# adobe/3D-FM-GAN

Measured on AMD Instinct MI355X. Metric: (photo,render) pairs/sec, higher is better.
Workload: dtype f32; 1 GPU; pairs1024: cfg4 shard: E_Tsr+E_W+E_W_Plus(18 styles) on 256^2 -> co-mod -> Generator(1024) forward, fp32, B=8/GPU; pairs_per_gpu=8, global_pairs=8, image_size=1024, parallelism=replicas x1 (batch-sharded, no collective), launch=eager, ranks=1, full=False

## Files before the change

3d-fm-gan_amd/csrc/live_weights.hip:

```cpp
#include "common.h"

namespace {

constexpr int LW_TO = 64, LW_TI = 16, LW_MAXT = 9;
constexpr int LW_ELEMS0 = 2048;

__global__ __launch_bounds__(256) void live_weights_f32(const fmgan_refresh_entry* __restrict__ table, int n_entries) {
  __shared__ float tile[LW_TO][LW_TI * LW_MAXT + 1];
  int lo = 0, hi = n_entries - 1;
  while (lo < hi) {
    const int mid = (lo + hi + 1) >> 1;
    if (table[mid].block_begin <= blockIdx.x) lo = mid; else hi = mid - 1;
  }
  const fmgan_refresh_entry e = table[lo];
  const unsigned lb = blockIdx.x - e.block_begin;
  const float* __restrict__ src = (const float*)e.src;
  float* __restrict__ dst = (float*)e.dst;
  if (e.kind == 0) {
    const long long base = (long long)lb * LW_ELEMS0;
#pragma unroll
    for (int k = 0; k < LW_ELEMS0 / 256; ++k) {
      const long long idx = base + threadIdx.x + 256 * k;
      if (idx < e.n) dst[idx] = src[idx] * e.scale;
    }
    return;
  }
  const int kt = e.ktaps, run = LW_TI * kt;
  const int i_tiles = (e.cin + LW_TI - 1) / LW_TI;
  const int o0 = (lb / i_tiles) * LW_TO, i0 = (lb % i_tiles) * LW_TI;
  const int i_n = min(LW_TI, e.cin - i0);
  for (int idx = threadIdx.x; idx < LW_TO * run; idx += 256) {
    const int o = idx / run, j = idx - o * run;
    float v = 0.f;
    if (o0 + o < e.cout && j < i_n * kt) v = src[((long long)(o0 + o) * e.cin + i0) * kt + j];
    tile[o][j] = v;
  }
  __syncthreads();
  for (int idx = threadIdx.x; idx < LW_TO * run; idx += 256) {
    const int j = idx / LW_TO, o = idx - j * LW_TO;
    if (o0 + o < e.cout && j < i_n * kt) dst[((long long)i0 * kt + j) * e.cout + o0 + o] = e.scale * tile[o][j];
  }
  float* __restrict__ wsq = (float*)e.dst2;
  if (wsq) {
    for (int idx = threadIdx.x; idx < LW_TO * LW_TI; idx += 256) {
      const int o = idx / LW_TI, i = idx % LW_TI;
      if (o0 + o < e.cout && i < i_n) {
        float q = 0.f;
        for (int t = 0; t < kt; ++t) { const float w = tile[o][i * kt + t]; q = fmaf(w, w, q); }
        wsq[(long long)(o0 + o) * e.cin + i0 + i] = q;
      }
    }
  }
}

}

extern "C" long long fmgan_weight_refresh_blocks(int kind, int cout, int cin, int ktaps, long long n) {
  if (kind == 0) return n > 0 ? (n + LW_ELEMS0 - 1) / LW_ELEMS0 : -1;
  if (kind == 1) {
    if (cout <= 0 || cin <= 0 || ktaps <= 0 || ktaps > LW_MAXT) return -1;
    return (long long)((cout + LW_TO - 1) / LW_TO) * ((cin + LW_TI - 1) / LW_TI);
  }
  return -1;
}

extern "C" int fmgan_weight_refresh_f32(const fmgan_refresh_entry* table_dev, int n_entries, long long total_blocks,
                                        void* stream) {
  if (n_entries < 0 || total_blocks < 0) return FMGAN_EINVAL;
  if (n_entries == 0 || total_blocks == 0) return FMGAN_OK;
  if (!table_dev) return FMGAN_EINVAL;
  if (total_blocks > 0x7fffffffLL) return FMGAN_EOVERFLOW;
  hipLaunchKernelGGL(live_weights_f32, dim3((unsigned)total_blocks), dim3(256), 0, (hipStream_t)stream, table_dev,
                     n_entries);
  return fmgan_check_launch();
}
```

3d-fm-gan_amd/csrc/winograd.hip:

```cpp
#include "common.h"

namespace {

__global__ __launch_bounds__(256) void wino_weight_f32(const float* __restrict__ wt, float* __restrict__ u, int cin, int cout) {
  const long long total = (long long)cin * cout;
  for (long long idx = (long long)blockIdx.x * blockDim.x + threadIdx.x; idx < total; idx += (long long)gridDim.x * blockDim.x) {
    const int i = (int)(idx % cin), o = (int)(idx / cin);
    float g[3][3];
#pragma unroll
    for (int t = 0; t < 9; ++t) g[t / 3][t % 3] = wt[((long long)i * 9 + t) * cout + o];
    float tmp[4][3];
#pragma unroll
    for (int k = 0; k < 3; ++k) {
      tmp[0][k] = g[0][k];
      tmp[1][k] = 0.5f * (g[0][k] + g[1][k] + g[2][k]);
      tmp[2][k] = 0.5f * (g[0][k] - g[1][k] + g[2][k]);
      tmp[3][k] = g[2][k];
    }
#pragma unroll
    for (int a = 0; a < 4; ++a) {
      const float uu[4] = {tmp[a][0], 0.5f * (tmp[a][0] + tmp[a][1] + tmp[a][2]), 0.5f * (tmp[a][0] - tmp[a][1] + tmp[a][2]),
                           tmp[a][2]};
#pragma unroll
      for (int bx = 0; bx < 4; ++bx) u[((long long)(a * 4 + bx) * cout + o) * cin + i] = uu[bx];
    }
  }
}

__global__ __launch_bounds__(256) void wino_input_f32(const float* __restrict__ x, const float* __restrict__ style,
                                                      float* __restrict__ v, int batch, int c, int h, int w) {
  const int tw = w >> 1, th = h >> 1, T = tw * th;
  const long long n_cols = (long long)batch * T, total = n_cols * c;
  for (long long idx = (long long)blockIdx.x * blockDim.x + threadIdx.x; idx < total; idx += (long long)gridDim.x * blockDim.x) {
    const int t = (int)(idx % T);
    const int ch = (int)((idx / T) % c);
    const int b = (int)(idx / ((long long)T * c));
    const int ty = t / tw, tx = t - ty * tw;
    const float* xp = x + ((long long)b * c + ch) * h * w;
    const float s = style[(long long)b * c + ch];
    float d[4][4];
#pragma unroll
    for (int r = 0; r < 4; ++r) {
      const int y = 2 * ty - 1 + r;
#pragma unroll
      for (int q = 0; q < 4; ++q) {
        const int xx = 2 * tx - 1 + q;
        d[r][q] = (y >= 0 && y < h && xx >= 0 && xx < w) ? xp[(long long)y * w + xx] * s : 0.f;
      }
    }
    float e[4][4];
#pragma unroll
    for (int r = 0; r < 4; ++r) {
      e[r][0] = d[r][0] - d[r][2]; e[r][1] = d[r][1] + d[r][2]; e[r][2] = d[r][2] - d[r][1]; e[r][3] = d[r][1] - d[r][3];
    }
    const long long col = (long long)b * T + t;
#pragma unroll
    for (int q = 0; q < 4; ++q) {
      const float v0 = e[0][q] - e[2][q], v1 = e[1][q] + e[2][q], v2 = e[2][q] - e[1][q], v3 = e[1][q] - e[3][q];
// ... 20 lines not shown
    const int ty = t / tw, tx = t - ty * tw;
    const long long col = (long long)b * T + t;
    float mm[4][4];
#pragma unroll
    for (int a = 0; a < 4; ++a)
#pragma unroll
      for (int q = 0; q < 4; ++q) mm[a][q] = m[((long long)(a * 4 + q) * cout + o) * n_cols + col];
    float z[2][4];
#pragma unroll
    for (int q = 0; q < 4; ++q) {
      z[0][q] = mm[0][q] + mm[1][q] + mm[2][q];
      z[1][q] = mm[1][q] - mm[2][q] - mm[3][q];
    }
    const float dm = demod ? demod[(long long)b * cout + o] : 1.f;
    const float bv = (fuse_act && bias) ? bias[o] : 0.f;
    float* op = out + (((long long)b * cout + o) * h + 2 * ty) * w + 2 * tx;
    const float* np = (fuse_act && noise) ? noise + ((long long)(noise_batch == 1 ? 0 : b) * h + 2 * ty) * w + 2 * tx : nullptr;
#pragma unroll
    for (int jy = 0; jy < 2; ++jy) {
      float y0 = (z[jy][0] + z[jy][1] + z[jy][2]) * dm, y1 = (z[jy][1] - z[jy][2] - z[jy][3]) * dm;
      if (fuse_act) {
        const float n0 = np ? __fmul_rn(nw, np[jy * w]) : 0.f, n1 = np ? __fmul_rn(nw, np[jy * w + 1]) : 0.f;
        y0 = __fadd_rn(__fadd_rn(y0, n0), bv);
        y1 = __fadd_rn(__fadd_rn(y1, n1), bv);
        y0 = (y0 > 0.f ? y0 : y0 * alpha) * act_scale;
        y1 = (y1 > 0.f ? y1 : y1 * alpha) * act_scale;
      }
      f32x2_u st; st.x = y0; st.y = y1;
      *reinterpret_cast<f32x2_u*>(op + (long long)jy * w) = st;
    }
  }
}

inline unsigned wino_grid(long long total) {
  long long blocks = (total + 255) / 256;
  const long long cap = (long long)FMGAN_NUM_CU * 32;
  if (blocks > cap) blocks = cap;
  return (unsigned)(blocks < 1 ? 1 : blocks);
}

}

extern "C" int fmgan_wino_weight_f32(const float* wt, float* u, int cin, int cout, void* stream) {
  if (cin <= 0 || cout <= 0) return FMGAN_EINVAL;
  if (!wt || !u) return FMGAN_EINVAL;
  hipLaunchKernelGGL(wino_weight_f32, dim3(wino_grid((long long)cin * cout)), dim3(256), 0, (hipStream_t)stream, wt, u, cin, cout);
  return fmgan_check_launch();
}

extern "C" int fmgan_wino_input_f32(const float* x, const float* style, float* v, int batch, int c, int h, int w, void* stream) {
  if (batch < 0 || c <= 0 || h <= 0 || w <= 0 || (h & 1) || (w & 1)) return FMGAN_EINVAL;
  if (batch == 0) return FMGAN_OK;
  if (!x || !style || !v) return FMGAN_EINVAL;
  hipLaunchKernelGGL(wino_input_f32, dim3(wino_grid((long long)batch * c * (h / 2) * (w / 2))), dim3(256), 0, (hipStream_t)stream,
                     x, style, v, batch, c, h, w);
  return fmgan_check_launch();
}

extern "C" int fmgan_wino_output_f32(const float* m, const float* demod, const float* noise, const float* noise_weight,
                                     const float* bias, float* out, int batch, int cout, int h, int w, int noise_batch,
                                     int fuse_act, float alpha, float act_scale, void* stream) {
  if (batch < 0 || cout <= 0 || h <= 0 || w <= 0 || (h & 1) || (w & 1)) return FMGAN_EINVAL;
  if (batch == 0) return FMGAN_OK;
  if (!m || !out) return FMGAN_EINVAL;
  if (fuse_act && noise && noise_batch != 1 && noise_batch != batch) return FMGAN_EINVAL;
  hipLaunchKernelGGL(wino_output_f32, dim3(wino_grid((long long)batch * cout * (h / 2) * (w / 2))), dim3(256), 0,
                     (hipStream_t)stream, m, demod, noise, noise_weight, bias, out, batch, cout, h, w, noise_batch, fuse_act, alpha,
                     act_scale);
  return fmgan_check_launch();
}
```

3d-fm-gan_amd/op/_native/__init__.py:

```python
from .core import (
    LIB_PATH, F32, F64, F16, BF16, FMGAN_OK, FMGAN_EINVAL, FMGAN_EUNSUPPORTED, amp_fwd, amp_bwd, lib, check, served,
    require_gpu, dtype_code, ptr, fp, require_f32_gpu, on_device, nhwc_dense, set_observer, launching)
from .activation import (
    activation_io, current_activation_io, io16, amp_fwd_io, BLUR_PATHS, upfirdn2d_out_size, upfirdn2d,
    upfirdn2d_strided, blur_noise_bias_act_serves, blur_noise_bias_act, fused_bias_act, fused_bias_act_backward,
    noise_bias_act, prelu_backward, dtype16_code, upfirdn2d16, fused_bias_act16, fused_bias_act16_backward)
from .conv import (
    modconv_demod, modconv_wsq, modconv_weight_prep, aligned_rows_shape, aligned_rows_buffer, modconv_precision,
    current_modconv_precision, modconv2d, modconv2d_rgb_fusable, modconv2d_select, modconv2d_tiles, modconv2d_rgb,
    modconv_weight_to_bf16, modconv_weight_to_bf16x3, conv_weight_to_bf16x3, conv3x3s2_bf16x3_supported,
    conv3x3s2_bf16x3, conv3x3_bf16x3_supported, conv3x3_bf16x3, C3_EPILOGUES, conv3x3_tail_bf16x3_select,
    conv3x3_tail_bf16x3, modconv_wgrad, modconv_wgrad_select, wino_weight,
    wino_input, wino_output, modconv2d_winograd, torgb,
    torgb_backward, equal_linear, style_bank, style_bank_concat, demod_bank)
from .encoder import bn_prelu, se_pool, se_gate, ir_tail
from .loss import (
    LPIPS_SIZE, face_region_loss, face_region_loss_backward, render_mask, lpips_distance, lpips_distance_backward,
    lpips_pair_input, projection_loss_fwd, projection_loss_bwd, HEATMAP_SIZE, face_crop_serves, face_crop_fwd,
    face_crop_bwd, detector_input, heatmap_distance_serves, heatmap_distance_fwd, heatmap_distance_bwd,
    landmark_decode)
from .evaluation import (
    face_input_pool, face_input, f64p, fid_stats_serves, fid_stats_update, fid_stats_finish, INCEPTION_SIZE,
    inception_input)
from .image import (
    images_to_tensor, resize_output_size, resize_plan, resize_images, tensor_to_images, tiles_to_canvas,
    BANK_GATHER_BANKS, BANK_GATHER_GROUPS, bank_gather)
from .optim import (
    lbfgs_segments, lbfgs_pair, lbfgs_coeffs, lbfgs_direction, lbfgs_update, lbfgs_gather, EMA_CHUNK,
    LOSS_ROW_COLUMNS, ema_blocks, ema, loss_row)
```

3d-fm-gan_amd/op/_native/conv.py:

```python
import ctypes

import torch

from .core import ambient, check, fp, launching, lib, nhwc_dense, _noise_args, on_device, ptr, require_gpu, served


def modconv_demod(weight, style, scale, eps=1e-8, wsq=None):
    cout, cin, kh, kw = weight.shape[-4:]
    style = style.contiguous()
    demod = torch.empty((style.shape[0], cout), dtype=torch.float32, device=style.device)
    with on_device(style) as stream:
        if wsq is not None:
            check(lib().fmgan_modconv_demod_wsq_f32(fp(wsq), fp(style), fp(demod), style.shape[0], cout, cin,
                                                    float(scale), float(eps), stream), 'modconv_demod_wsq')
        else:
            check(lib().fmgan_modconv_demod_f32(fp(weight), fp(style), fp(demod), style.shape[0], cout, cin,
                                                kh * kw, float(scale), float(eps), stream), 'modconv_demod')
    return demod


def modconv_wsq(weight):
    cout, cin, kh, kw = weight.shape[-4:]
    wsq = torch.empty((cout, cin), dtype=torch.float32, device=weight.device)
    with on_device(weight) as stream:
# ... 206 lines not shown
    with launching(x, 'conv3x3_tail_bf16x3', (b, cin, cout, h, w)) as stream:
        st = lib().fmgan_conv3x3_tail_bf16x3_f32(fp(x), ptr(wts), fp(bias), fp(out), b, cin, cout, h, w, float(alpha),
                                                 int(bool(channels_last)), stream)
    return out if served(st, 'conv3x3_tail_bf16x3') else None


def modconv_wgrad(go, demod, x, style, scale, fast_only=False, mode=0):
    go, x, style = go.contiguous(), x.contiguous(), style.contiguous()
    b, cout = go.shape[:2]
    cin, h, w = x.shape[1:]
    if (fast_only or mode != 0) and (cin < 48 or cout < 48):
        return None
    ws_bytes = lib().fmgan_modconv_wgrad_mode_workspace_bytes(b, cin, cout, h, w, int(mode))
    if ws_bytes == 0:
        return None
    ws = torch.empty(ws_bytes // 4, dtype=torch.float32, device=x.device)
    gw = torch.empty((cout, cin, 3, 3), dtype=torch.float32, device=x.device)
    with launching(x, 'modconv_wgrad', (b, cin, cout, h, w, int(mode))) as stream:
        st = lib().fmgan_modconv_wgrad_mode_f32(fp(go), fp(demod), fp(x), fp(style), fp(gw), b, cin, cout, h, w,
                                                int(mode), float(scale), fp(ws), ws_bytes, stream)
    check(st, 'modconv_wgrad')
    return gw


def modconv_wgrad_select(batch, cin, cout, h, w, mode=0, aligned16=True):
    v = [ctypes.c_int() for _ in range(7)]
    st = lib().fmgan_modconv_wgrad_select(int(batch), int(cin), int(cout), int(h), int(w), int(mode), int(bool(aligned16)),
                                          *[ctypes.byref(c) for c in v])
    served(st, 'modconv_wgrad_select')
    family, tw, sp, ks, tps, ntiles, vec = (c.value for c in v)
    return family, tw, sp, ks, tps, ntiles, bool(vec)


def wino_weight(wt):
    cin, taps, cout = wt.shape
    if taps != 9:
        raise RuntimeError('wino_weight: 3x3 weights only')
    u = torch.empty((16, cout, cin), dtype=torch.float32, device=wt.device)
    with on_device(wt) as stream:
        check(lib().fmgan_wino_weight_f32(fp(wt), fp(u), cin, cout, stream), 'wino_weight')
    return u


def wino_input(x, style):
    require_gpu(x, 'input')
    x, style = x.contiguous(), style.contiguous()
    b, cin, h, w = x.shape
    v = torch.empty((16, cin, b * (h // 2) * (w // 2)), dtype=torch.float32, device=x.device)
    with on_device(x) as stream:
        check(lib().fmgan_wino_input_f32(fp(x), fp(style), fp(v), b, cin, h, w, stream), 'wino_input')
    return v


def wino_output(m, demod, batch, h, w, noise=None, noise_weight=None, bias=None, fuse_act=False, alpha=0.2,
                act_scale=2 ** 0.5):
    require_gpu(m, 'm')
    m = m.contiguous()
    cout = m.shape[1]
    if m.shape[0] != 16 or m.shape[2] != batch * (h // 2) * (w // 2):
        raise RuntimeError('wino_output: M must be [16, cout, B*(H/2)*(W/2)]')
    out = torch.empty((batch, cout, h, w), dtype=torch.float32, device=m.device)
    nz, nb = _noise_args(noise)
    with on_device(m) as stream:
        check(lib().fmgan_wino_output_f32(fp(m), fp(demod), fp(nz), fp(noise_weight), fp(bias), fp(out), batch, cout, h, w,
                                          nb, int(bool(fuse_act)), float(alpha), float(act_scale), stream), 'wino_output')
    return out
# ... 98 lines not shown
```

3d-fm-gan_amd/op/_native/core.py:

```python
import ctypes
import os

import torch

_PKG = os.path.dirname(os.path.dirname(os.path.dirname(os.path.abspath(__file__))))
LIB_PATH = os.environ.get('FMGAN_LIB') or os.path.join(_PKG, 'csrc', 'libfmgan_hip.so')

F32, F64, F16 = 0, 1, 2
BF16 = 3
FMGAN_OK, FMGAN_EINVAL, FMGAN_EUNSUPPORTED = 0, -1, -2
_DTYPES = {torch.float32: F32, torch.float64: F64, torch.float16: F16}

_lib = None

amp_fwd = torch.amp.custom_fwd(device_type='cuda', cast_inputs=torch.float32)
amp_bwd = torch.amp.custom_bwd(device_type='cuda')


class ambient:
    values, text, scope, var = (), '', None, ''

    def __init__(self, value):
        if value not in self.values:
            raise ValueError(self.text)
# ... 45 lines not shown
    _sig(L.fmgan_act16_fba_bwd_blocks, [ll, i])
    _sig(L.fmgan_act16_fba_bwd, [i] + [vp] * 4 + [ll, i, f, f, vp])
    _sig(L.fmgan_ufd16_select, [i] * 15)
    _sig(L.fmgan_ufd16, [i, vp, vp, vp] + [i] * 14 + [vp])
    _sig(L.fmgan_modconv_demod_f32, [vp] * 3 + [i] * 4 + [f, f, vp])
    _sig(L.fmgan_modconv_wsq_f32, [vp] * 2 + [i] * 3 + [vp])
    _sig(L.fmgan_modconv_demod_wsq_f32, [vp] * 3 + [i] * 3 + [f, f, vp])
    _sig(L.fmgan_modconv_weight_prep_f32, [vp, vp, i, i, i, f, i, vp])
    _sig(L.fmgan_modconv2d_workspace_bytes, [i] * 6, ll)
    _sig(L.fmgan_modconv2d_f32, [vp] * 5 + [i] * 6 + [vp] * 3 + [i, i, f, f, ll, i, vp, ll, vp])
    _sig(L.fmgan_modconv2d_rgb_fusable, [i] * 5)
    _sig(L.fmgan_modconv2d_select, [i] * 8 + [ctypes.POINTER(i)] * 5)
    _sig(L.fmgan_modconv2d_tiles, [ctypes.POINTER(i), i])
    _sig(L.fmgan_modconv2d_rgb_f32, [vp] * 5 + [i] * 5 + [vp] * 3 + [i, i, f, f] + [vp] * 4 + [i, vp])
    _sig(L.fmgan_modconv_weight_bf16_bytes, [i] * 3, ll)
    _sig(L.fmgan_modconv_weight_to_bf16, [vp, vp, i, i, i, vp])
    _sig(L.fmgan_modconv2d_bf16_supported, [i] * 6)
    _sig(L.fmgan_modconv2d_bf16, [vp] * 5 + [i] * 6 + [vp] * 3 + [i, i, f, f, ll, i, vp])
    _sig(L.fmgan_modconv_weight_bf16x3_bytes, [i] * 3, ll)
    _sig(L.fmgan_modconv_weight_to_bf16x3, [vp, vp, i, i, i, vp])
    _sig(L.fmgan_modconv2d_bf16x3_supported, [i] * 6)
    _sig(L.fmgan_modconv2d_bf16x3, [vp] * 5 + [i] * 6 + [vp] * 3 + [i, i, f, f, ll, i, vp])
    _sig(L.fmgan_conv3x3s2_bf16x3_supported, [i] * 5)
    _sig(L.fmgan_conv3x3s2_bf16x3_f32, [vp] * 4 + [i] * 5 + [f, i, vp])
    _sig(L.fmgan_conv3x3_bf16x3_supported, [i] * 7)
    _sig(L.fmgan_conv3x3_bf16x3_f32, [vp] * 4 + [i] * 9 + [f, vp])
    _sig(L.fmgan_conv3x3_tail_bf16x3_select, [i] * 5)
    _sig(L.fmgan_conv3x3_tail_bf16x3_f32, [vp] * 4 + [i] * 5 + [f, i, vp])
    _sig(L.fmgan_modconv_wgrad_workspace_bytes, [i] * 5, ll)
    _sig(L.fmgan_modconv_wgrad_f32, [vp] * 5 + [i] * 5 + [f, vp, ll, vp])
    _sig(L.fmgan_modconv_wgrad_mode_workspace_bytes, [i] * 6, ll)
    _sig(L.fmgan_modconv_wgrad_mode_f32, [vp] * 5 + [i] * 6 + [f, vp, ll, vp])
    _sig(L.fmgan_modconv_wgrad_select, [i] * 7 + [ctypes.POINTER(i)] * 7)
    _sig(L.fmgan_wino_weight_f32, [vp, vp, i, i, vp])
    _sig(L.fmgan_wino_input_f32, [vp] * 3 + [i] * 4 + [vp])
    _sig(L.fmgan_wino_output_f32, [vp] * 6 + [i] * 6 + [f, f, vp])
    _sig(L.fmgan_torgb_weight_mod_f32, [vp] * 3 + [i] * 3 + [f, vp])
    _sig(L.fmgan_torgb_f32, [vp] * 6 + [i] * 4 + [f, vp])
    _sig(L.fmgan_torgb_backward_splits, [i] * 3)
    _sig(L.fmgan_torgb_backward_f32, [vp] * 6 + [i] * 4 + [f, vp])
    _sig(L.fmgan_equal_linear_f32, [vp] * 4 + [i] * 3 + [vp])
    _sig(L.fmgan_style_bank_entry_bytes, [])
    _sig(L.fmgan_style_bank_f32, [vp, i, vp, vp, i, i, i, vp, vp])
    _sig(L.fmgan_style_bank_concat_f32, [vp, i, vp, vp, i, i, i, i, vp, vp])
    _sig(L.fmgan_demod_bank_f32, [vp, i, vp, i, vp, vp])
    _sig(L.fmgan_weight_refresh_blocks, [i, i, i, i, ll], ll)
    _sig(L.fmgan_weight_refresh_f32, [vp, i, ll, vp])
    _sig(L.fmgan_bn_prelu_f32, [vp] * 5 + [f, vp, vp] + [vp] * 4 + [f, vp, vp] + [i] * 5 + [vp])
    _sig(L.fmgan_se_pool_chunks, [i] * 4)
    _sig(L.fmgan_se_pool_f32, [vp, vp] + [i] * 4 + [vp])
    _sig(L.fmgan_se_gate_f32, [vp, i, ll] + [vp] * 4 + [f] + [vp] * 3 + [i] * 3 + [vp])
    _sig(L.fmgan_ir_tail_f32, [vp] * 5 + [f, vp, vp] + [i] * 3 + [vp] * 4 + [f, vp] + [vp] * 4 + [f, vp] + [i] * 4 + [vp])
    _sig(L.fmgan_face_region_blocks, [i, ll])
    _sig(L.fmgan_face_region_loss_f32, [vp] * 3 + [i, i, ll, vp])
    _sig(L.fmgan_face_region_backward_f32, [vp] * 4 + [i, i, ll, vp])
    _sig(L.fmgan_render_mask_f32, [vp] * 2 + [i, i, ll, vp])
    _sig(L.fmgan_lpips_distance_blocks, [i] * 3)
    _sig(L.fmgan_lpips_distance_f32, [vp] * 4 + [i, i, i, f, vp])
    _sig(L.fmgan_lpips_distance_backward_f32, [vp] * 6 + [i, i, i, f, vp])
    _sig(L.fmgan_lpips_pair_input_select, [i] * 8)
    _sig(L.fmgan_lpips_pair_input_f32, [vp] * 5 + [i] * 8 + [vp])
    _sig(L.fmgan_projection_loss_select, [i] * 4)
    _sig(L.fmgan_projection_loss_blocks, [i] * 4)
    _sig(L.fmgan_projection_loss_fwd_f32, [vp] * 7 + [i] * 4 + [vp])
    _sig(L.fmgan_projection_loss_bwd_f32, [vp] * 7 + [i] * 4 + [vp])
    _sig(L.fmgan_face_crop_select, [i] * 4)
# ... 156 lines not shown
```

3d-fm-gan_amd/op/live_weights.py:

```python
import weakref

import numpy as np
import torch

from . import _native

_ENTRY = np.dtype([('src', '<u8'), ('dst', '<u8'), ('dst2', '<u8'), ('n', '<i8'), ('kind', '<i4'), ('cout', '<i4'),
                   ('cin', '<i4'), ('ktaps', '<i4'), ('scale', '<f4'), ('block_begin', '<u4')])


def _check_layout():
    if _native.lib().fmgan_refresh_entry_bytes() != _ENTRY.itemsize:
        raise RuntimeError('fmgan_refresh_entry layout mismatch between libfmgan_hip.so and op/live_weights.py')


class LiveWeights:

    def __init__(self, root):
        self.root = root
        self.active = False
        self._key = None
        self._table = None
        self._blocks = 0
        self._n = 0
        self._buffers = []

    def __deepcopy__(self, memo):
        import copy
        new = LiveWeights.__new__(LiveWeights)
        memo[id(self)] = new
        new.__init__(copy.deepcopy(self.root, memo))
        return new

    def _sources(self):
        from stylegan2 import EqualLinear, ModulatedConv2d
        lin, conv = [], []
        for m in self.root.modules():
            if isinstance(m, EqualLinear):
                lin.append(m)
            elif isinstance(m, ModulatedConv2d) and m.kernel_size == 3:
                conv.append(m)
        return lin, conv

    def _build(self, lin, conv, key):
        _check_layout()
        rows, bufs = [], []
        blocks = 0

        def add(kind, src, dst, dst2, cout, cin, ktaps, scale, n):
            nonlocal blocks
            nb = _native.lib().fmgan_weight_refresh_blocks(kind, cout, cin, ktaps, n)
            if nb <= 0:
                raise RuntimeError('live_weights: unsupported entry')
            rows.append((src.data_ptr(), dst.data_ptr(), 0 if dst2 is None else dst2.data_ptr(), n, kind, cout, cin,
                         ktaps, scale, blocks))
            blocks += nb

        for m in lin:
            w = m.weight
            ws = torch.empty_like(w, memory_format=torch.contiguous_format)
            bs = None
            add(0, w, ws, None, 0, 0, 0, m.scale, w.numel())
            if m.bias is not None:
                bs = torch.empty_like(m.bias)
                add(0, m.bias, bs, None, 0, 0, 0, m.lr_mul, m.bias.numel())
            m._live = (self, ws, bs)
            bufs += [ws, bs]
        for m in conv:
            w = m.weight
            cout, cin, k, _ = w.shape[-4:]
            wt = torch.empty((cin, k * k, cout), dtype=torch.float32, device=w.device)
            wsq = torch.empty((cout, cin), dtype=torch.float32, device=w.device)
            add(1, w, wt, wsq, cout, cin, k * k, m.scale, 0)
            m._live = (self, wt, wsq)
            bufs += [wt, wsq]
        table = np.array(rows, dtype=_ENTRY)
        dev = (lin[0].weight if lin else conv[0].weight).device
        self._table = torch.from_numpy(table.view(np.uint8).copy()).to(dev)
        self._blocks, self._n, self._buffers, self._key = blocks, len(rows), bufs, key

    def refresh(self):
        lin, conv = self._sources()
        if not lin and not conv:
            return False
        params = [m.weight for m in lin + conv] + [m.bias for m in lin if m.bias is not None]
        if any((not p.is_cuda) or p.dtype != torch.float32 or not p.is_contiguous() for p in params):
            return False
        key = tuple((p.data_ptr(), p.device.index) for p in params)
        if key != self._key:
            self._build(lin, conv, key)
        with _native.on_device(self._table) as stream:
            _native.check(_native.lib().fmgan_weight_refresh_f32(self._table.data_ptr(), self._n, self._blocks, stream),
                          'weight_refresh')
        return True

    def fresh(self):
        return _Fresh(self)


class _Fresh:
    def __init__(self, lw):
        self.lw = lw

    def __enter__(self):
        self.prev = self.lw.active
        if not self.prev:
            self.lw.active = self.lw.refresh()
        return self.lw

    def __exit__(self, *exc):
        self.lw.active = self.prev
        return False


def live(module):
    lv = getattr(module, '_live', None)
    if lv is not None and lv[0].active and not torch.is_grad_enabled():
        return lv[1], lv[2]
    return None


_SPLIT = weakref.WeakKeyDictionary()


def split_conv_weight(conv, bracket='conv_weight_bf16x3'):
    w = conv.weight
    key = (w.data_ptr(), w._version, w.device, tuple(w.shape), tuple(w.stride()))
    kept = _SPLIT.get(conv)
    stream = torch.cuda.current_stream(w.device)
    if kept is None or kept[0] != key:
        img = _native.conv_weight_to_bf16x3(w, bracket)
        built = torch.cuda.Event()
        built.record(stream)
        kept = (key, img, built, stream)
        _SPLIT[conv] = kept
    elif kept[3] != stream:
        stream.wait_event(kept[2])
    return kept[1]


def drop_split_weight(conv=None):
    if conv is None:
        _SPLIT.clear()
    else:
        _SPLIT.pop(conv, None)
```

3d-fm-gan_amd/stylegan2.py:

```python
import math
import os
import random

import torch
from torch import nn, autograd
from torch.nn import functional as F

from op import FusedLeakyReLU, fused_leaky_relu, upfirdn2d
from op import _native, conv_grad, modconv, placement
from op._native import amp_fwd as _amp_fwd, amp_bwd as _amp_bwd
from op.live_weights import LiveWeights, live
from op.style_bank import Modulation, StyleBank, comod_column, concat_column, sliced_columns
from Util.streams import side_streams, run_on, overlap_ok

_SQRT2 = math.sqrt(2.0)


def _channel_table(channel_multiplier):
    table = {4: 512, 8: 512, 16: 512, 32: 512}
    for res, base in ((64, 256), (128, 128), (256, 64), (512, 32), (1024, 16)):
        table[res] = base * channel_multiplier
    return table


def make_kernel(k):
    k = torch.as_tensor(k, dtype=torch.float32)
    if k.ndim == 1:
        k = torch.outer(k, k)
    return k / k.sum()


class PixelNorm(nn.Module):

    def forward(self, input):
        return input * torch.rsqrt(input.square().mean(dim=1, keepdim=True) + 1e-8)


class Upsample(nn.Module):

    def __init__(self, kernel, factor=2):
        super().__init__()
        self.factor = factor
        self.register_buffer('kernel', make_kernel(kernel) * (factor ** 2))
        p = self.kernel.shape[0] - factor
# ... 89 lines not shown
    def forward(self, input):
        return F.leaky_relu(input, negative_slope=self.negative_slope) * _SQRT2


def _fir_pads(n_taps, kernel_size, upsample):
    if upsample:
        p = (n_taps - 2) - (kernel_size - 1)
        return (p + 1) // 2 + 1, p // 2 + 1
    p = (n_taps - 2) + (kernel_size - 1)
    return (p + 1) // 2, p // 2


class ModulatedConv2d(nn.Module):

    def __init__(self, in_channel, out_channel, kernel_size, style_dim, demodulate=True, upsample=False,
                 downsample=False, blur_kernel=[1, 3, 3, 1]):
        super().__init__()
        self.eps = 1e-8
        self.kernel_size = kernel_size
        self.in_channel = in_channel
        self.out_channel = out_channel
        self.upsample = upsample
        self.downsample = downsample
        if upsample:
            self.blur = Blur(blur_kernel, pad=_fir_pads(len(blur_kernel), kernel_size, True), upsample_factor=2)
        if downsample:
            self.blur = Blur(blur_kernel, pad=_fir_pads(len(blur_kernel), kernel_size, False))
        self.scale = 1 / math.sqrt(in_channel * kernel_size ** 2)
        self.padding = kernel_size // 2
        self.weight = nn.Parameter(torch.randn(1, out_channel, in_channel, kernel_size, kernel_size))
        self.modulation = EqualLinear(style_dim, in_channel, bias_init=1)
        self.demodulate = demodulate
        self._live = None

    def __repr__(self):
        return (f'{self.__class__.__name__}({self.in_channel}, {self.out_channel}, {self.kernel_size}, '
                f'upsample={self.upsample}, downsample={self.downsample})')

    def mfma_weight(self):
        lv = live(self)
        if lv is not None:
            return lv[0]
        with torch.no_grad():
            return _native.modconv_weight_prep(self.weight.detach(), self.scale)

    def mfma_wsq(self):
        lv = live(self)
        if lv is not None:
            return lv[1]
        with torch.no_grad():
            return _native.modconv_wsq(self.weight.detach())

    def styles(self, style):
        return self.modulation(style)

    def forward(self, input, style, return_style_scalars=False):
        s = self.styles(style)
        hip = modconv.hip_conv_ok(input, self.weight)
        wt = self.mfma_weight() if hip else None
        if self.upsample:
            out = self.blur(modconv.modulated_conv2d(input, self.weight, s, wt, self.demodulate, 1, self.scale))
        elif self.downsample:
            out = modconv.modulated_conv2d(self.blur(input), self.weight, s, wt, self.demodulate, 2, self.scale)
        else:
            out = modconv.modulated_conv2d(input, self.weight, s, wt, self.demodulate, 0, self.scale)
        if return_style_scalars:
            return out, s.view(s.shape[0], 1, self.in_channel, 1, 1)
        return out


class _NoiseInjectionFunction(autograd.Function):

    @staticmethod
    @_amp_fwd
    def forward(ctx, image, weight, noise):
        ctx.save_for_backward(weight, noise)
        return image + weight * noise

    @staticmethod
    @_amp_bwd
    def backward(ctx, go):
        weight, noise = ctx.saved_tensors
        g_weight = g_noise = None
        if ctx.needs_input_grad[1] or ctx.needs_input_grad[2]:
# ... 91 lines not shown
                                               conv.blur.kernel, (pad0, pad1), noise, self.noise.weight, act.bias,
                                               act.negative_slope, act.scale, out=out)
        nbytes = 4 * shape[0] * shape[1] * shape[2]
        ws = None
        if (placement.active() and nbytes >= placement.MIN_BYTES
                and _native.blur_noise_bias_act_serves(b, c, 2 * h + 1, 2 * w + 1, ps, rs, conv.blur.kernel.shape,
                                                       (pad0, pad1))):
            ws = placement.workspace(self, (b, c, h, w), shape, (b, c, 2 * h, 2 * w), input.device, produce, consume)
        if ws is not None:
            produce(ws.buf)
            if consume(ws.buf, ws.out) is None:
                raise RuntimeError('StyledConv: the fused blur declined a shape its selection reported as served')
            return ws.out
        buf = torch.empty(shape, dtype=torch.float32, device=input.device)
        produce(buf)
        out = consume(buf, None)
        if out is None:
            out = _native.upfirdn2d_strided(buf.data_ptr() + 4 * off, input.device, b * c, 2 * h + 1, 2 * w + 1, ps,
                                            rs, conv.blur.kernel, pad0, pad1, pad0, pad1).view(b, c, 2 * h, 2 * w)
            out = _native.noise_bias_act(out, noise, self.noise.weight, act.bias, act.negative_slope, act.scale)
        return out

    def _fused(self, input, style, noise):
        conv, act = self.conv, self.activate
        s, demod = _modulation(conv, style)
        b, _, h, w = input.shape
        if noise is None:
            noise = input.new_empty(b, 1, *((2 * h, 2 * w) if conv.upsample else (h, w))).normal_()
        if conv.upsample:
            out = self._fused_upsample(input, s, demod, noise)
        elif winograd_pays(b, conv.in_channel, conv.out_channel, h, w):
            out = _native.modconv2d_winograd(input, conv.mfma_weight(), s, demod, noise=noise,
                                             noise_weight=self.noise.weight, bias=act.bias, fuse_act=True,
                                             alpha=act.negative_slope, act_scale=act.scale)
        else:
            out = _native.modconv2d(input, conv.mfma_weight(), s, demod, 0, noise=noise,
                                    noise_weight=self.noise.weight, bias=act.bias, fuse_act=True,
                                    alpha=act.negative_slope, act_scale=act.scale)
        return out, s

    def rgb_fusable(self, x_shape, x):
        conv = self.conv
        if conv.upsample or conv.downsample or torch.is_grad_enabled() or not modconv.hip_conv_ok(x, conv.weight):
            return False
        if _native.current_modconv_precision() != 'f32':
            return False
        b, _, h, w = x_shape
        return _native.modconv2d_rgb_fusable(b, conv.in_channel, conv.out_channel, h, w)

    def fused_with_rgb(self, input, style, noise, to_rgb, rgb_style, skip_up, keep_out):
        return _fp32(self._fused_with_rgb, input, style, noise, to_rgb, rgb_style, skip_up, keep_out)

    def _fused_with_rgb(self, input, style, noise, to_rgb, rgb_style, skip_up, keep_out):
        conv, act = self.conv, self.activate
        s, demod = _modulation(conv, style)
        rgb_s = _modulation(to_rgb.conv, rgb_style).style
        if noise is None:
            noise = input.new_empty(input.shape[0], 1, input.shape[2], input.shape[3]).normal_()
        return _native.modconv2d_rgb(input, conv.mfma_weight(), s, demod, noise, self.noise.weight, act.bias,
                                     act.negative_slope, act.scale, to_rgb.conv.weight, rgb_s,
                                     to_rgb.bias, skip_up, to_rgb.conv.scale, keep_out)

    def forward(self, input, style, return_style_scalars=False, noise=None):
        fused = (not torch.is_grad_enabled()) and modconv.hip_conv_ok(input, self.conv.weight) and not self.conv.downsample
        if isinstance(style, Modulation) and not fused:
            raise RuntimeError('StyledConv: precomputed styles serve the fused inference path on float32 GPU tensors only')
        if fused:
# ... 356 lines not shown
```

include/fmgan_hip.h:

```cpp
#ifndef FMGAN_HIP_H
#define FMGAN_HIP_H

#ifdef __cplusplus
extern "C" {
#endif

#define FMGAN_ABI_VERSION 1

#define FMGAN_OK            0
#define FMGAN_EINVAL       -1
#define FMGAN_EUNSUPPORTED -2
#define FMGAN_ELAUNCH      -3
#define FMGAN_EOVERFLOW    -4

#define FMGAN_F32 0
#define FMGAN_F64 1
#define FMGAN_F16 2
#define FMGAN_BF16 3

int         fmgan_abi_version(void);
const char *fmgan_status_string(int status);

int fmgan_upfirdn2d_select(int dtype, int major, int in_h, int in_w, int minor,
                           int kernel_h, int kernel_w, int up_x, int up_y,
// ... 99 lines not shown
int fmgan_heatmap_distance_fwd_f32(const float *a, const float *b, float *partial, int batch, long long m, void *stream);
int fmgan_heatmap_distance_bwd_f32(const float *a, const float *b, const float *g, float *grad_a, float *grad_b, int batch,
                                   long long m, void *stream);
int fmgan_landmark_decode_f32(const float *hm, const float *center, const float *scale, float *preds, float *preds_orig,
                              int batch, int channels, int h, int w, void *stream);

int fmgan_bn_prelu_f32(const float *x, const float *mean, const float *var, const float *gamma, const float *beta,
                       float eps, const float *slope, float *y, const float *next_mean, const float *next_var,
                       const float *next_gamma, const float *next_beta, float next_eps, float *y_next, float *y_sub,
                       int batch, int channels, int h, int w, int sub_stride, void *stream);
int fmgan_se_pool_chunks(int batch, int channels, int h, int w);
int fmgan_se_pool_f32(const float *r, float *partial, int batch, int channels, int h, int w, void *stream);
int fmgan_se_gate_f32(const float *partial, int chunks, long long hw, const float *mean, const float *var,
                      const float *gamma, const float *beta, float eps, const float *fc1, const float *fc2, float *gate,
                      int batch, int channels, int mid, void *stream);
int fmgan_ir_tail_f32(const float *r, const float *mean, const float *var, const float *gamma, const float *beta,
                      float eps, const float *gate, const float *shortcut, int sc_h, int sc_w, int sc_stride,
                      const float *sc_mean, const float *sc_var, const float *sc_gamma, const float *sc_beta, float sc_eps,
                      float *out, const float *next_mean, const float *next_var, const float *next_gamma,
                      const float *next_beta, float next_eps, float *out_next, int batch, int channels, int h, int w,
                      void *stream);

int fmgan_lpips_distance_blocks(int batch, int channels, int hw);
int fmgan_lpips_distance_f32(const float *f0, const float *f1, const float *w, float *partial, int batch, int channels,
                             int hw, float eps, void *stream);
int fmgan_lpips_distance_backward_f32(const float *f0, const float *f1, const float *w, const float *grad,
                                      float *grad_f0, float *grad_f1, int batch, int channels, int hw, float eps,
                                      void *stream);

int fmgan_modconv_demod_f32(const float *weight, const float *style, float *demod,
                            int batch, int cout, int cin, int ktaps,
                            float scale, float eps, void *stream);

int fmgan_wino_weight_f32(const float *wt, float *u, int cin, int cout, void *stream);
int fmgan_wino_input_f32(const float *x, const float *style, float *v, int batch, int c, int h, int w, void *stream);
int fmgan_wino_output_f32(const float *m, const float *demod, const float *noise, const float *noise_weight,
                          const float *bias, float *out, int batch, int cout, int h, int w, int noise_batch,
                          int fuse_act, float alpha, float act_scale, void *stream);

int fmgan_equal_linear_f32(const float *x, const float *weight, const float *bias, float *out,
                           int batch, int n_out, int k_in, void *stream);

int fmgan_modconv_wsq_f32(const float *weight, float *wsq, int cout, int cin, int ktaps, void *stream);
int fmgan_modconv_demod_wsq_f32(const float *wsq, const float *style, float *demod,
                                int batch, int cout, int cin, float scale, float eps, void *stream);

int fmgan_modconv_weight_prep_f32(const float *weight, float *wt, int cout, int cin, int ktaps,
                                  float scale, int kind, void *stream);

typedef struct fmgan_refresh_entry {
  const void *src;
  void *dst;
  void *dst2;
  long long n;
  int kind, cout, cin, ktaps;
  float scale;
  unsigned block_begin;
} fmgan_refresh_entry;
int fmgan_refresh_entry_bytes(void);
long long fmgan_weight_refresh_blocks(int kind, int cout, int cin, int ktaps, long long n);
int fmgan_weight_refresh_f32(const fmgan_refresh_entry *table_dev, int n_entries, long long total_blocks,
                             void *stream);

typedef struct fmgan_style_bank_entry {
  const void *ws;
  const void *bs;
  const void *wsq;
  long long style_off, demod_off;
  int col, sliced, n_styles, cin, cout, demodulate;
  float scale, eps;
} fmgan_style_bank_entry;
int fmgan_style_bank_entry_bytes(void);
int fmgan_style_bank_f32(const fmgan_style_bank_entry *table_dev, int n_entries, const float *w, const float *wplus,
                         int wplus_batch, int batch, int style_dim, float *styles_out, void *stream);
int fmgan_style_bank_concat_f32(const fmgan_style_bank_entry *table_dev, int n_entries, const float *v,
                                const float *wplus, int wplus_batch, int batch, int dv, int dw, float *styles_out,
                                void *stream);
int fmgan_demod_bank_f32(const fmgan_style_bank_entry *table_dev, int n_entries, const float *styles, int batch,
                         float *demod_out, void *stream);

long long fmgan_modconv2d_workspace_bytes(int batch, int cin, int cout, int h, int w, int mode);
int fmgan_modconv2d_f32(const float *in, const float *wt, const float *style,
                        const float *demod, float *out,
                        int batch, int cin, int cout, int h, int w, int mode,
                        const float *noise, const float *noise_weight, const float *bias,
                        int noise_batch, int fuse_act, float alpha, float act_scale,
// ... 134 lines not shown
```

Before: 443.3 pairs/s.

## Fuse Winograd weight transform into live weight refresh and vectorize transforms

For eligible 3x3 modulated convs with at least 256 channels, the live-weight refresh kernel now also writes the Winograd-transformed weights U from its shared tile. This removes a separate wino_weight pass per forward. The standalone weight transform is re-tiled through shared memory so its reads coalesce. New strip kernels handle four tiles per thread with 16-byte vector loads and stores for the input and output transforms, selected when width and alignment allow. The cost is extra buffer memory and a larger refresh kernel, and it relies on modconv2d_winograd accepting a precomputed u.

```diff
diff --git a/3d-fm-gan_amd/csrc/live_weights.hip b/3d-fm-gan_amd/csrc/live_weights.hip
--- a/3d-fm-gan_amd/csrc/live_weights.hip
+++ b/3d-fm-gan_amd/csrc/live_weights.hip
@@ -1,4 +1,5 @@
 #include "common.h"
+#include "winograd_weight.h"
 
 namespace {
 
@@ -51,6 +52,20 @@
       }
     }
   }
+  float* __restrict__ u = (float*)e.dst3;
+  if (u && kt == 9) {
+    for (int idx = threadIdx.x; idx < LW_TO * LW_TI; idx += 256) {
+      const int o = idx / LW_TI, i = idx % LW_TI;
+      if (o0 + o < e.cout && i < i_n) {
+        float g[3][3], uu[16];
+#pragma unroll
+        for (int t = 0; t < 9; ++t) g[t / 3][t % 3] = e.scale * tile[o][i * 9 + t];
+        wino_weight_transform(g, uu);
+#pragma unroll
+        for (int xi = 0; xi < 16; ++xi) u[((long long)xi * e.cout + o0 + o) * e.cin + i0 + i] = uu[xi];
+      }
+    }
+  }
 }
 
 }
diff --git a/3d-fm-gan_amd/csrc/winograd.hip b/3d-fm-gan_amd/csrc/winograd.hip
--- a/3d-fm-gan_amd/csrc/winograd.hip
+++ b/3d-fm-gan_amd/csrc/winograd.hip
@@ -1,29 +1,33 @@
 #include "common.h"
+#include "winograd_weight.h"
 
 namespace {
 
+constexpr int WW_T = 16;
+
 __global__ __launch_bounds__(256) void wino_weight_f32(const float* __restrict__ wt, float* __restrict__ u, int cin, int cout) {
-  const long long total = (long long)cin * cout;
-  for (long long idx = (long long)blockIdx.x * blockDim.x + threadIdx.x; idx < total; idx += (long long)gridDim.x * blockDim.x) {
-    const int i = (int)(idx % cin), o = (int)(idx / cin);
-    float g[3][3];
-#pragma unroll
-    for (int t = 0; t < 9; ++t) g[t / 3][t % 3] = wt[((long long)i * 9 + t) * cout + o];
-    float tmp[4][3];
-#pragma unroll
-    for (int k = 0; k < 3; ++k) {
-      tmp[0][k] = g[0][k];
-      tmp[1][k] = 0.5f * (g[0][k] + g[1][k] + g[2][k]);
-      tmp[2][k] = 0.5f * (g[0][k] - g[1][k] + g[2][k]);
-      tmp[3][k] = g[2][k];
-    }
-#pragma unroll
-    for (int a = 0; a < 4; ++a) {
-      const float uu[4] = {tmp[a][0], 0.5f * (tmp[a][0] + tmp[a][1] + tmp[a][2]), 0.5f * (tmp[a][0] - tmp[a][1] + tmp[a][2]),
-                           tmp[a][2]};
-#pragma unroll
-      for (int bx = 0; bx < 4; ++bx) u[((long long)(a * 4 + bx) * cout + o) * cin + i] = uu[bx];
-    }
+  __shared__ float taps[9][WW_T][WW_T + 1];
+  const int i_tiles = (cin + WW_T - 1) / WW_T, o_tiles = (cout + WW_T - 1) / WW_T;
+  const long long tiles = (long long)i_tiles * o_tiles;
+  for (long long tile = blockIdx.x; tile < tiles; tile += gridDim.x) {
+    const int i0 = (int)(tile % i_tiles) * WW_T, o0 = (int)(tile / i_tiles) * WW_T;
+    for (int idx = threadIdx.x; idx < 9 * WW_T * WW_T; idx += 256) {
+      const int ol = idx % WW_T, r = idx / WW_T, il = r / 9, t = r - il * 9;
+      if (i0 + il < cin && o0 + ol < cout) taps[t][il][ol] = wt[((long long)(i0 + il) * 9 + t) * cout + o0 + ol];
+    }
+    __syncthreads();
+    for (int idx = threadIdx.x; idx < WW_T * WW_T; idx += 256) {
+      const int il = idx % WW_T, ol = idx / WW_T;
+      if (i0 + il < cin && o0 + ol < cout) {
+        float g[3][3], uu[16];
+#pragma unroll
+        for (int t = 0; t < 9; ++t) g[t / 3][t % 3] = taps[t][il][ol];
+        wino_weight_transform(g, uu);
+#pragma unroll
+        for (int xi = 0; xi < 16; ++xi) u[((long long)xi * cout + o0 + ol) * cin + i0 + il] = uu[xi];
+      }
+    }
+    __syncthreads();
   }
 }
 
@@ -110,40 +114,172 @@
   }
 }
 
-inline unsigned wino_grid(long long total) {
-  long long blocks = (total + 255) / 256;
-  const long long cap = (long long)FMGAN_NUM_CU * 32;
+
+__global__ __launch_bounds__(256) void wino_input_strip_f32(const float* __restrict__ x, const float* __restrict__ style,
+                                                            float* __restrict__ v, int batch, int c, int h, int w) {
+  const int tw = w >> 1, th = h >> 1, T = tw * th, sw = tw >> 2;
+  const long long n_cols = (long long)batch * T, total = (long long)batch * c * th * sw;
+  for (long long idx = (long long)blockIdx.x * blockDim.x + threadIdx.x; idx < total; idx += (long long)gridDim.x * blockDim.x) {
+    const int sx = (int)(idx % sw);
+    const int ty = (int)((idx / sw) % th);
+    const int ch = (int)((idx / ((long long)sw * th)) % c);
+    const int b = (int)(idx / ((long long)sw * th * c));
+    const int x0 = 8 * sx;
+    const bool left = x0 > 0, right = x0 + 8 < w;
+    const float* xp = x + ((long long)b * c + ch) * h * w + x0;
+    const float s = style[(long long)b * c + ch];
+    float e[4][4][4];
+#pragma unroll
+    for (int r = 0; r < 4; ++r) {
+      const int y = 2 * ty - 1 + r;
+      const bool in = y >= 0 && y < h;
+      const float* row = xp + (long long)(in ? y : 0) * w;
+      const f32x4 lo = *reinterpret_cast<const f32x4*>(row), hi = *reinterpret_cast<const f32x4*>(row + 4);
+      const float raw[10] = {row[left ? -1 : 0], lo.x, lo.y, lo.z, lo.w, hi.x, hi.y, hi.z, hi.w, row[right ? 8 : 7]};
+      float d[10];
+#pragma unroll
+      for (int q = 0; q < 10; ++q) {
+        const bool ok = in && (q > 0 || left) && (q < 9 || right);
+        d[q] = ok ? raw[q] * s : 0.f;
+      }
+#pragma unroll
+      for (int k = 0; k < 4; ++k) {
+        e[r][k][0] = d[2 * k] - d[2 * k + 2]; e[r][k][1] = d[2 * k + 1] + d[2 * k + 2];
+        e[r][k][2] = d[2 * k + 2] - d[2 * k + 1]; e[r][k][3] = d[2 * k + 1] - d[2 * k + 3];
+      }
+    }
+    const long long col = (long long)b * T + (long long)ty * tw + 4 * sx;
+#pragma unroll
+    for (int q = 0; q < 4; ++q) {
+      f32x4 v0, v1, v2, v3;
+#pragma unroll
+      for (int k = 0; k < 4; ++k) {
+        v0[k] = e[0][k][q] - e[2][k][q]; v1[k] = e[1][k][q] + e[2][k][q];
+        v2[k] = e[2][k][q] - e[1][k][q]; v3[k] = e[1][k][q] - e[3][k][q];
+      }
+      *reinterpret_cast<f32x4*>(v + ((long long)(0 * 4 + q) * c + ch) * n_cols + col) = v0;
+      *reinterpret_cast<f32x4*>(v + ((long long)(1 * 4 + q) * c + ch) * n_cols + col) = v1;
+      *reinterpret_cast<f32x4*>(v + ((long long)(2 * 4 + q) * c + ch) * n_cols + col) = v2;
+      *reinterpret_cast<f32x4*>(v + ((long long)(3 * 4 + q) * c + ch) * n_cols + col) = v3;
+    }
+  }
+}
+
+__global__ __launch_bounds__(256) void wino_output_strip_f32(const float* __restrict__ m, const float* __restrict__ demod,
+                                                             const float* __restrict__ noise,
+                                                             const float* __restrict__ noise_weight,
+                                                             const float* __restrict__ bias, float* __restrict__ out, int batch,
+                                                             int cout, int h, int w, int noise_batch, int fuse_act, float alpha,
+                                                             float act_scale) {
+  const int tw = w >> 1, th = h >> 1, T = tw * th, sw = tw >> 2;
+  const long long n_cols = (long long)batch * T, total = (long long)batch * cout * th * sw;
+  const float nw = (fuse_act && noise && noise_weight) ? noise_weight[0] : 0.f;
+  for (long long idx = (long long)blockIdx.x * blockDim.x + threadIdx.x; idx < total; idx += (long long)gridDim.x * blockDim.x) {
+    const int sx = (int)(idx % sw);
+    const int ty = (int)((idx / sw) % th);
+    const int o = (int)((idx / ((long long)sw * th)) % cout);
+    const int b = (int)(idx / ((long long)sw * th * cout));
+    const long long col = (long long)b * T + (long long)ty * tw + 4 * sx;
+    f32x4 mm[4][4];
+#pragma unroll
+    for (int a = 0; a < 4; ++a)
+#pragma unroll
+      for (int q = 0; q < 4; ++q) mm[a][q] = *reinterpret_cast<const f32x4*>(m + ((long long)(a * 4 + q) * cout + o) * n_cols + col);
+    const float dm = demod ? demod[(long long)b * cout + o] : 1.f;
+    const float bv = (fuse_act && bias) ? bias[o] : 0.f;
+    float* op = out + (((long long)b * cout + o) * h + 2 * ty) * w + 8 * sx;
+    const float* np = (fuse_act && noise) ? noise + ((long long)(noise_batch == 1 ? 0 : b) * h + 2 * ty) * w + 8 * sx : nullptr;
+#pragma unroll
+    for (int jy = 0; jy < 2; ++jy) {
+      float nz[8] = {0.f, 0.f, 0.f, 0.f, 0.f, 0.f, 0.f, 0.f};
+      if (fuse_act && np) {
+        const f32x4 lo = *reinterpret_cast<const f32x4*>(np + (long long)jy * w);
+        const f32x4 hi = *reinterpret_cast<const f32x4*>(np + (long long)jy * w + 4);
+#pragma unroll
+        for (int k = 0; k < 4; ++k) { nz[k] = __fmul_rn(nw, lo[k]); nz[4 + k] = __fmul_rn(nw, hi[k]); }
+      }
+      float y[8];
+#pragma unroll
+      for (int k = 0; k < 4; ++k) {
+        float z[4];
+#pragma unroll
+        for (int q = 0; q < 4; ++q)
+          z[q] = jy == 0 ? mm[0][q][k] + mm[1][q][k] + mm[2][q][k] : mm[1][q][k] - mm[2][q][k] - mm[3][q][k];
+        float y0 = (z[0] + z[1] + z[2]) * dm, y1 = (z[1] - z[2] - z[3]) * dm;
+        if (fuse_act) {
+          y0 = __fadd_rn(__fadd_rn(y0, nz[2 * k]), bv);
+          y1 = __fadd_rn(__fadd_rn(y1, nz[2 * k + 1]), bv);
+          y0 = (y0 > 0.f ? y0 : y0 * alpha) * act_scale;
+          y1 = (y1 > 0.f ? y1 : y1 * alpha) * act_scale;
+        }
+        y[2 * k] = y0; y[2 * k + 1] = y1;
+      }
+      const f32x4 s0 = {y[0], y[1], y[2], y[3]}, s1 = {y[4], y[5], y[6], y[7]};
+      *reinterpret_cast<f32x4*>(op + (long long)jy * w) = s0;
+      *reinterpret_cast<f32x4*>(op + (long long)jy * w + 4) = s1;
+    }
+  }
+}
+
+inline unsigned wino_grid(long long tiles, int per_thread = 1) {
+  long long blocks = (tiles / per_thread + 255) / 256;
+  const long long cap = (long long)FMGAN_NUM_CU * 32 / per_thread;
   if (blocks > cap) blocks = cap;
   return (unsigned)(blocks < 1 ? 1 : blocks);
 }
 
+inline bool aligned16(const void* p) { return ((uintptr_t)p & 15) == 0; }
+
+inline int wino_kernel(bool output, int w, bool all_aligned16) {
+  return ((w >> 1) & 3) == 0 && all_aligned16 && !(output && w < 32) ? 1 : 0;
+}
+
+inline int wino_sizes(int batch, int c, int h, int w) {
+  return (batch < 0 || c <= 0 || h <= 0 || w <= 0 || (h & 1) || (w & 1)) ? FMGAN_EINVAL : FMGAN_OK;
+}
+
+}
+
+extern "C" int fmgan_wino_select(int output, int batch, int c, int h, int w, int all_aligned16) {
+  const int st = wino_sizes(batch, c, h, w);
+  return st != FMGAN_OK ? st : wino_kernel(output != 0, w, all_aligned16 != 0);
 }
 
 extern "C" int fmgan_wino_weight_f32(const float* wt, float* u, int cin, int cout, void* stream) {
   if (cin <= 0 || cout <= 0) return FMGAN_EINVAL;
   if (!wt || !u) return FMGAN_EINVAL;
-  hipLaunchKernelGGL(wino_weight_f32, dim3(wino_grid((long long)cin * cout)), dim3(256), 0, (hipStream_t)stream, wt, u, cin, cout);
+  long long blocks = (long long)((cin + WW_T - 1) / WW_T) * ((cout + WW_T - 1) / WW_T);
+  if (blocks > (long long)FMGAN_NUM_CU * 32) blocks = (long long)FMGAN_NUM_CU * 32;
+  hipLaunchKernelGGL(wino_weight_f32, dim3((unsigned)blocks), dim3(256), 0, (hipStream_t)stream, wt, u, cin, cout);
   return fmgan_check_launch();
 }
 
 extern "C" int fmgan_wino_input_f32(const float* x, const float* style, float* v, int batch, int c, int h, int w, void* stream) {
-  if (batch < 0 || c <= 0 || h <= 0 || w <= 0 || (h & 1) || (w & 1)) return FMGAN_EINVAL;
+  if (wino_sizes(batch, c, h, w) != FMGAN_OK) return FMGAN_EINVAL;
   if (batch == 0) return FMGAN_OK;
   if (!x || !style || !v) return FMGAN_EINVAL;
-  hipLaunchKernelGGL(wino_input_f32, dim3(wino_grid((long long)batch * c * (h / 2) * (w / 2))), dim3(256), 0, (hipStream_t)stream,
-                     x, style, v, batch, c, h, w);
+  const long long tiles = (long long)batch * c * (h / 2) * (w / 2);
+  if (wino_kernel(false, w, aligned16(x) && aligned16(v)))
+    hipLaunchKernelGGL(wino_input_strip_f32, dim3(wino_grid(tiles, 4)), dim3(256), 0, (hipStream_t)stream, x, style, v, batch, c,
+                       h, w);
+  else
+    hipLaunchKernelGGL(wino_input_f32, dim3(wino_grid(tiles)), dim3(256), 0, (hipStream_t)stream, x, style, v, batch, c, h, w);
   return fmgan_check_launch();
 }
 
 extern "C" int fmgan_wino_output_f32(const float* m, const float* demod, const float* noise, const float* noise_weight,
                                      const float* bias, float* out, int batch, int cout, int h, int w, int noise_batch,
                                      int fuse_act, float alpha, float act_scale, void* stream) {
-  if (batch < 0 || cout <= 0 || h <= 0 || w <= 0 || (h & 1) || (w & 1)) return FMGAN_EINVAL;
+  if (wino_sizes(batch, cout, h, w) != FMGAN_OK) return FMGAN_EINVAL;
   if (batch == 0) return FMGAN_OK;
   if (!m || !out) return FMGAN_EINVAL;
   if (fuse_act && noise && noise_batch != 1 && noise_batch != batch) return FMGAN_EINVAL;
-  hipLaunchKernelGGL(wino_output_f32, dim3(wino_grid((long long)batch * cout * (h / 2) * (w / 2))), dim3(256), 0,
-                     (hipStream_t)stream, m, demod, noise, noise_weight, bias, out, batch, cout, h, w, noise_batch, fuse_act, alpha,
-                     act_scale);
+  const long long tiles = (long long)batch * cout * (h / 2) * (w / 2);
+  if (wino_kernel(true, w, aligned16(m) && aligned16(out) && (!(fuse_act && noise) || aligned16(noise))))
+    hipLaunchKernelGGL(wino_output_strip_f32, dim3(wino_grid(tiles, 4)), dim3(256), 0, (hipStream_t)stream, m, demod, noise,
+                       noise_weight, bias, out, batch, cout, h, w, noise_batch, fuse_act, alpha, act_scale);
+  else
+    hipLaunchKernelGGL(wino_output_f32, dim3(wino_grid(tiles)), dim3(256), 0, (hipStream_t)stream, m, demod, noise, noise_weight,
+                       bias, out, batch, cout, h, w, noise_batch, fuse_act, alpha, act_scale);
   return fmgan_check_launch();
 }
diff --git a/3d-fm-gan_amd/csrc/winograd_weight.h b/3d-fm-gan_amd/csrc/winograd_weight.h
--- /dev/null
+++ b/3d-fm-gan_amd/csrc/winograd_weight.h
@@ -0,0 +1,19 @@
+#pragma once
+
+__device__ __forceinline__ void wino_weight_transform(const float (&g)[3][3], float (&u)[16]) {
+  float tmp[4][3];
+#pragma unroll
+  for (int k = 0; k < 3; ++k) {
+    tmp[0][k] = g[0][k];
+    tmp[1][k] = 0.5f * (g[0][k] + g[1][k] + g[2][k]);
+    tmp[2][k] = 0.5f * (g[0][k] - g[1][k] + g[2][k]);
+    tmp[3][k] = g[2][k];
+  }
+#pragma unroll
+  for (int a = 0; a < 4; ++a) {
+    u[a * 4 + 0] = tmp[a][0];
+    u[a * 4 + 1] = 0.5f * (tmp[a][0] + tmp[a][1] + tmp[a][2]);
+    u[a * 4 + 2] = 0.5f * (tmp[a][0] - tmp[a][1] + tmp[a][2]);
+    u[a * 4 + 3] = tmp[a][2];
+  }
+}
diff --git a/3d-fm-gan_amd/op/_native/__init__.py b/3d-fm-gan_amd/op/_native/__init__.py
--- a/3d-fm-gan_amd/op/_native/__init__.py
+++ b/3d-fm-gan_amd/op/_native/__init__.py
@@ -10,7 +10,7 @@
     current_modconv_precision, modconv2d, modconv2d_rgb_fusable, modconv2d_select, modconv2d_tiles, modconv2d_rgb,
     modconv_weight_to_bf16, modconv_weight_to_bf16x3, conv_weight_to_bf16x3, conv3x3s2_bf16x3_supported,
     conv3x3s2_bf16x3, conv3x3_bf16x3_supported, conv3x3_bf16x3, C3_EPILOGUES, conv3x3_tail_bf16x3_select,
-    conv3x3_tail_bf16x3, modconv_wgrad, modconv_wgrad_select, wino_weight,
+    conv3x3_tail_bf16x3, modconv_wgrad, modconv_wgrad_select, wino_select, wino_weight,
     wino_input, wino_output, modconv2d_winograd, torgb,
     torgb_backward, equal_linear, style_bank, style_bank_concat, demod_bank)
 from .encoder import bn_prelu, se_pool, se_gate, ir_tail
diff --git a/3d-fm-gan_amd/op/_native/conv.py b/3d-fm-gan_amd/op/_native/conv.py
--- a/3d-fm-gan_amd/op/_native/conv.py
+++ b/3d-fm-gan_amd/op/_native/conv.py
@@ -262,6 +262,13 @@
     return family, tw, sp, ks, tps, ntiles, bool(vec)
 
 
+def wino_select(transform, batch, c, h, w, *tensors):
+    aligned = all(t.data_ptr() % 16 == 0 for t in tensors if t is not None)
+    k = lib().fmgan_wino_select(('input', 'output').index(transform), int(batch), int(c), int(h), int(w), int(aligned))
+    check(min(k, 0), 'wino_select')
+    return ('tile', 'strip')[k]
+
+
 def wino_weight(wt):
     cin, taps, cout = wt.shape
     if taps != 9:
diff --git a/3d-fm-gan_amd/op/_native/core.py b/3d-fm-gan_amd/op/_native/core.py
--- a/3d-fm-gan_amd/op/_native/core.py
+++ b/3d-fm-gan_amd/op/_native/core.py
@@ -101,6 +101,7 @@
     _sig(L.fmgan_modconv_wgrad_mode_workspace_bytes, [i] * 6, ll)
     _sig(L.fmgan_modconv_wgrad_mode_f32, [vp] * 5 + [i] * 6 + [f, vp, ll, vp])
     _sig(L.fmgan_modconv_wgrad_select, [i] * 7 + [ctypes.POINTER(i)] * 7)
+    _sig(L.fmgan_wino_select, [i] * 6)
     _sig(L.fmgan_wino_weight_f32, [vp, vp, i, i, vp])
     _sig(L.fmgan_wino_input_f32, [vp] * 3 + [i] * 4 + [vp])
     _sig(L.fmgan_wino_output_f32, [vp] * 6 + [i] * 6 + [f, f, vp])
diff --git a/3d-fm-gan_amd/op/live_weights.py b/3d-fm-gan_amd/op/live_weights.py
--- a/3d-fm-gan_amd/op/live_weights.py
+++ b/3d-fm-gan_amd/op/live_weights.py
@@ -5,8 +5,9 @@
 
 from . import _native
 
-_ENTRY = np.dtype([('src', '<u8'), ('dst', '<u8'), ('dst2', '<u8'), ('n', '<i8'), ('kind', '<i4'), ('cout', '<i4'),
-                   ('cin', '<i4'), ('ktaps', '<i4'), ('scale', '<f4'), ('block_begin', '<u4')])
+_ENTRY = np.dtype([('src', '<u8'), ('dst', '<u8'), ('dst2', '<u8'), ('dst3', '<u8'), ('n', '<i8'), ('kind', '<i4'),
+                   ('cout', '<i4'), ('cin', '<i4'), ('ktaps', '<i4'), ('scale', '<f4'), ('block_begin', '<u4')])
+WINOGRAD_MIN_CHANNELS = 256
 
 
 def _check_layout():
@@ -43,17 +44,18 @@
         return lin, conv
 
     def _build(self, lin, conv, key):
+        from stylegan2 import WINOGRAD
         _check_layout()
         rows, bufs = [], []
         blocks = 0
 
-        def add(kind, src, dst, dst2, cout, cin, ktaps, scale, n):
+        def add(kind, src, dst, dst2, cout, cin, ktaps, scale, n, dst3=None):
             nonlocal blocks
             nb = _native.lib().fmgan_weight_refresh_blocks(kind, cout, cin, ktaps, n)
             if nb <= 0:
                 raise RuntimeError('live_weights: unsupported entry')
-            rows.append((src.data_ptr(), dst.data_ptr(), 0 if dst2 is None else dst2.data_ptr(), n, kind, cout, cin,
-                         ktaps, scale, blocks))
+            rows.append((src.data_ptr(), dst.data_ptr(), 0 if dst2 is None else dst2.data_ptr(),
+                         0 if dst3 is None else dst3.data_ptr(), n, kind, cout, cin, ktaps, scale, blocks))
             blocks += nb
 
         for m in lin:
@@ -71,9 +73,13 @@
             cout, cin, k, _ = w.shape[-4:]
             wt = torch.empty((cin, k * k, cout), dtype=torch.float32, device=w.device)
             wsq = torch.empty((cout, cin), dtype=torch.float32, device=w.device)
-            add(1, w, wt, wsq, cout, cin, k * k, m.scale, 0)
+            u = None
+            if WINOGRAD and k == 3 and not (m.upsample or m.downsample) and min(cin, cout) >= WINOGRAD_MIN_CHANNELS:
+                u = torch.empty((16, cout, cin), dtype=torch.float32, device=w.device)
+            add(1, w, wt, wsq, cout, cin, k * k, m.scale, 0, u)
             m._live = (self, wt, wsq)
-            bufs += [wt, wsq]
+            m._live_u = u
+            bufs += [wt, wsq, u]
         table = np.array(rows, dtype=_ENTRY)
         dev = (lin[0].weight if lin else conv[0].weight).device
         self._table = torch.from_numpy(table.view(np.uint8).copy()).to(dev)
@@ -120,6 +126,10 @@
     return None
 
 
+def live_u(module):
+    return getattr(module, '_live_u', None) if live(module) is not None else None
+
+
 _SPLIT = weakref.WeakKeyDictionary()
 
 
diff --git a/3d-fm-gan_amd/stylegan2.py b/3d-fm-gan_amd/stylegan2.py
--- a/3d-fm-gan_amd/stylegan2.py
+++ b/3d-fm-gan_amd/stylegan2.py
@@ -9,7 +9,7 @@
 from op import FusedLeakyReLU, fused_leaky_relu, upfirdn2d
 from op import _native, conv_grad, modconv, placement
 from op._native import amp_fwd as _amp_fwd, amp_bwd as _amp_bwd
-from op.live_weights import LiveWeights, live
+from op.live_weights import LiveWeights, live, live_u
 from op.style_bank import Modulation, StyleBank, comod_column, concat_column, sliced_columns
 from Util.streams import side_streams, run_on, overlap_ok
 
@@ -165,6 +165,7 @@
         self.modulation = EqualLinear(style_dim, in_channel, bias_init=1)
         self.demodulate = demodulate
         self._live = None
+        self._live_u = None
 
     def __repr__(self):
         return (f'{self.__class__.__name__}({self.in_channel}, {self.out_channel}, {self.kernel_size}, '
@@ -183,6 +184,9 @@
             return lv[1]
         with torch.no_grad():
             return _native.modconv_wsq(self.weight.detach())
+
+    def wino_weight(self):
+        return live_u(self)
 
     def styles(self, style):
         return self.modulation(style)
@@ -340,7 +344,7 @@
         elif winograd_pays(b, conv.in_channel, conv.out_channel, h, w):
             out = _native.modconv2d_winograd(input, conv.mfma_weight(), s, demod, noise=noise,
                                              noise_weight=self.noise.weight, bias=act.bias, fuse_act=True,
-                                             alpha=act.negative_slope, act_scale=act.scale)
+                                             alpha=act.negative_slope, act_scale=act.scale, u=conv.wino_weight())
         else:
             out = _native.modconv2d(input, conv.mfma_weight(), s, demod, 0, noise=noise,
                                     noise_weight=self.noise.weight, bias=act.bias, fuse_act=True,
diff --git a/include/fmgan_hip.h b/include/fmgan_hip.h
--- a/include/fmgan_hip.h
+++ b/include/fmgan_hip.h
@@ -155,6 +155,7 @@
                             int batch, int cout, int cin, int ktaps,
                             float scale, float eps, void *stream);
 
+int fmgan_wino_select(int output, int batch, int c, int h, int w, int all_aligned16);
 int fmgan_wino_weight_f32(const float *wt, float *u, int cin, int cout, void *stream);
 int fmgan_wino_input_f32(const float *x, const float *style, float *v, int batch, int c, int h, int w, void *stream);
 int fmgan_wino_output_f32(const float *m, const float *demod, const float *noise, const float *noise_weight,
@@ -175,6 +176,7 @@
   const void *src;
   void *dst;
   void *dst2;
+  void *dst3;
   long long n;
   int kind, cout, cin, ktaps;
   float scale;
```

Measured after the change: 448.9 pairs/s (median of 6 runs). 1.3% higher.
